# Enigmatisms/AdaPT

Measured on AMD Instinct MI355X. Metric: Msamples/s (W*H*spp/s), unidirectional MIS path tracing, higher is better.
Workload: dtype f32

## Files before the change

### adapt_amd/csrc/rng.hpp

```cpp
#pragma once
#include "vec.hpp"
#include <stdint.h>

struct Philox {
    uint32_t key0, key1, ctr0;
    uint32_t draw;
    uint32_t blk;
    uint32_t nblk;
    uint32_t c[4], n[4];
};

APT_HD void philox4x32_10(uint32_t c0, uint32_t c1, uint32_t c2, uint32_t c3, uint32_t k0, uint32_t k1, uint32_t out[4]) {
#if defined(__HIP_DEVICE_COMPILE__)
    asm volatile("" : "+v"(k0));
#endif
#pragma unroll
    for (int r = 0; r < 10; r++) {
        uint64_t p0 = (uint64_t)0xD2511F53u * c0;
        uint64_t p1 = (uint64_t)0xCD9E8D57u * c2;
        uint32_t n0 = (uint32_t)(p1 >> 32) ^ c1 ^ k0;
        uint32_t n1 = (uint32_t)p1;
        uint32_t n2 = (uint32_t)(p0 >> 32) ^ c3 ^ k1;
        uint32_t n3 = (uint32_t)p0;
        c0 = n0; c1 = n1; c2 = n2; c3 = n3;
        k0 += 0x9E3779B9u; k1 += 0xBB67AE85u;
    }
    out[0] = c0; out[1] = c1; out[2] = c2; out[3] = c3;
}

APT_HD void rng_init(Philox& r, uint32_t pixel, uint32_t seed, uint32_t sample, uint32_t draw) {
    r.key0 = pixel; r.key1 = seed; r.ctr0 = sample; r.draw = draw; r.blk = 0xffffffffu; r.nblk = 0xffffffffu;
    r.c[0] = r.c[1] = r.c[2] = r.c[3] = 0u;
    r.n[0] = r.n[1] = r.n[2] = r.n[3] = 0u;
}
APT_HD uint32_t rng_u32(Philox& r) {
    const uint32_t d = r.draw++;
    const uint32_t b = d >> 2;
    const bool step = b != r.blk;
    if (step && b != r.nblk) { philox4x32_10(r.ctr0, b, 0u, 0u, r.key0, r.key1, r.n); r.nblk = b; }
    if (step) { r.c[0] = r.n[0]; r.c[1] = r.n[1]; r.c[2] = r.n[2]; r.c[3] = r.n[3]; r.blk = b; r.nblk = 0xffffffffu; }
    const uint32_t w = d & 3u, c0 = r.c[0], c1 = r.c[1], c2 = r.c[2], c3 = r.c[3];
    return (w == 0u) ? c0 : ((w == 1u) ? c1 : ((w == 2u) ? c2 : c3));
}
APT_HD void rng_open(Philox& r) {
    const uint32_t b = r.draw >> 2;
    philox4x32_10(r.ctr0, b, 0u, 0u, r.key0, r.key1, r.c); r.blk = b;
    philox4x32_10(r.ctr0, b + 1u, 0u, 0u, r.key0, r.key1, r.n); r.nblk = b + 1u;
}
APT_HD float rng_float(Philox& r) { return (float)(rng_u32(r) >> 8) * (1.0f / 16777216.0f); }
APT_HD int32_t rng_int(Philox& r) { return (int32_t)rng_u32(r); }
APT_HD int pymod(int a, int n) { int m = a % n; return (m < 0) ? m + n : m; }
```

### adapt_amd/csrc/shade_stage.hpp

```cpp
#pragma once
#include "stages.hpp"

APT_D float ti_fmod(float a, float b) { float q = floorf(a / b); return a - b * q; }
APT_D f3 mix3(f3 a, f3 b, float t) { return a * (1.0f - t) + b * t; }
APT_D f3 texture_query(const DevScene& sc, int map, int obj, float u, float v) {
    const int* ti_ = sc.tex_i + 15 * obj + 5 * map; const float* tf = sc.tex_f + 6 * obj + 2 * map;
    const float w = (float)ti_[3], h = (float)ti_[4];
    const float scaled_u = ti_fmod((u * tf[0]) * w, w - 1.f), scaled_v = ti_fmod((v * tf[1]) * h, h - 1.f);
    float floor_u = floorf(scaled_u), floor_v = floorf(scaled_v);
    const float ratio_u = scaled_u - floor_u, ratio_v = scaled_v - floor_v;
    floor_u = floor_u + (float)ti_[1]; floor_v = floor_v + (float)ti_[2];
    const int fu = (int)floor_u, fv = (int)floor_v;
    const float* img = sc.atlas[map]; const int W = sc.atlas_w[map];
    const float* r0 = img + ((size_t)fv * W + fu) * 3; const float* r1 = r0 + (size_t)W * 3;
    const f3 q_ff = mk3(r0[0], r0[1], r0[2]), q_cf = mk3(r0[3], r0[4], r0[5]), q_fc = mk3(r1[0], r1[1], r1[2]), q_cc = mk3(r1[3], r1[4], r1[5]);
    return mix3(mix3(q_ff, q_cf, ratio_u), mix3(q_fc, q_cc, ratio_u), ratio_v);
}
APT_D bool get_uv_item(const DevScene& sc, int map, int obj, int prim, float bu, float bv, f3& out) {
    if (sc.atlas[map] == nullptr || !(sc.tex_i[15 * obj + 5 * map] > -255)) return false;
    const float* uv = sc.uvs + 6 * prim;
    const float w0 = 1.f - bu - bv;
    const float gu = (uv[2] * bu + uv[4] * bv) + uv[0] * w0, gv = (uv[3] * bu + uv[5] * bv) + uv[1] * w0;
    out = texture_query(sc, map, obj, gu, gv);
    return true;
// ... 83 lines not shown
    }
    flush_stat(t_lit, &cnt->stats[sq][ST_LIT]);
    if (lane_id() == 0) __hip_atomic_store(n_sh_p, 0u, __ATOMIC_RELAXED, __HIP_MEMORY_SCOPE_AGENT);
    __threadfence();
    if (lane_id() == 0) __hip_atomic_store(&cnt->fix_done[sq * CNT_PAD], epoch, __ATOMIC_RELEASE, __HIP_MEMORY_SCOPE_AGENT);
}
#endif
#ifndef APT_ARGS_RELOAD
#define APT_ARGS_RELOAD 1
#endif
struct ShadeArgs3 { DevScene sc; Params p; Queues q; };
typedef const __attribute__((address_space(4))) ShadeArgs3* args3_ptr;
APT_D args3_ptr kernel_args3() { return (args3_ptr)__builtin_amdgcn_kernarg_segment_ptr(); }
APT_D const ShadeArgs3* args_fresh(args3_ptr a) {
#if APT_ARGS_RELOAD
    asm volatile("" : "+s"(a));
#endif
    return (const ShadeArgs3*)a;
}
#if APT_ARGS_RELOAD
#define APT_ARGS_PHASE() (A_ = args_fresh(A0))
#else
#define APT_ARGS_PHASE() ((void)0)
#endif
struct Vertex {
    f3 o, d, thr, hit_point; uint32_t id, l_off, draw0; float emission_weight;
    Hit it; int hit_light; DevBxdf bx;
};
APT_D void vertex_reset(Vertex& vx) {
    vx.o = splat3(0.f); vx.d = mk3(0.f, 0.f, 1.f); vx.thr = splat3(0.f); vx.hit_point = splat3(0.f); vx.id = 0; vx.l_off = 0; vx.draw0 = 0; vx.emission_weight = 1.0f;
    vx.it.obj_id = -1; vx.it.prim_id = -1; vx.it.n_s = vx.it.n_g = mk3(1.f, 0.f, 0.f); vx.it.min_depth = 0.f; vx.hit_light = -1;
    vx.bx.type = 1; vx.bx.is_delta = 0; vx.bx.is_bsdf = 0; vx.bx.k_d = vx.bx.k_s = vx.bx.k_g = vx.bx.mean = splat3(0.f); vx.bx.ior = 1.f;
}
template <int BM, int SM, int TEX>
APT_D bool open_vertex(const ShadeArgs3* A_, Vertex& vx, Philox& rng, int prim, f3 rec_kd, uint32_t meta, float ray_pdf, float2 uv, int bounce) {
    const bool was_spec = (meta >> 24) & 1u;
    if (BM == 0x002) vx.bx.k_d = rec_kd;
    else vx.bx = ld_bxdf_lane((A_->sc).bxdf + vx.it.obj_id);
    if (TEX && (A_->sc).tex_i != nullptr) {
        f3 tx;
        if (bounce == 0) {
            if (get_uv_item((A_->sc), 1, vx.it.obj_id, prim, uv.x, uv.y, tx)) { m33 R; rotation_between(mk3(0.f, 1.f, 0.f), vx.it.n_g, R); vx.it.n_s = mul(R, tx); }
            if (get_uv_item((A_->sc), 2, vx.it.obj_id, prim, uv.x, uv.y, tx)) vx.it.n_s = delocalize(vx.it.n_s, tx);
        }
        if (get_uv_item((A_->sc), 0, vx.it.obj_id, prim, uv.x, uv.y, tx)) vx.bx.k_d = tx;
    }
    const uint32_t lp = vx.id & ((1u << (A_->p).pix_bits) - 1u), s = vx.id >> (A_->p).pix_bits;
    vx.l_off = (s * (uint32_t)(A_->p).npix + lp) << 2;
    vx.draw0 = meta & 0xffffu;
    rng_init(rng, ((A_->p).world == 1) ? lp : ldq((A_->p).pix_key, lp << 2), (A_->p).seed, (uint32_t)((A_->p).cnt_base + (int)s + 1), vx.draw0);
    if (bounce > 0 && (A_->p).use_mis) {
        float e_pdf = 0.0f;
        if (vx.hit_light >= 0 && vx.bx.is_delta == 0 && !was_spec) e_pdf = emitter_solid_angle_pdf((A_->sc).src[vx.hit_light], vx.it, vx.d);
        vx.emission_weight = balance(ray_pdf, e_pdf);
    }
    if (!(SM & 2)) rng_open(rng);
    if ((A_->p).use_rr) {
        float mx = max3(vx.thr);
        if (mx < (A_->p).rr_threshold && bounce >= (A_->p).rr_bounce_th) {
            if (rng_float(rng) > mx) return false;
            vx.thr = vx.thr * srcp(mx + 1e-7f);
        }
    } else if (max3(vx.thr) < 1e-4f) return false;
    return true;
}
struct LightSample { bool want, sampled, poisoned; f3 dir, contrib; float dist, mis_w; int src; };
template <int BM, int SM, bool LANE_SRC>
APT_D LightSample sample_light(const ShadeArgs3* A_, Vertex& vx, Philox& rng, const EmitterGeom& geom, const DevSrc src_only, bool active, bool& break_flag) {
    LightSample ls; ls.want = ls.sampled = ls.poisoned = false; ls.dir = ls.contrib = splat3(0.f); ls.dist = 0.f; ls.mis_w = 1.0f; ls.src = 0;
    if (!active || break_flag) return ls;
    const int ns = (A_->sc).n_sources;
    int sidx = rng_int(rng);
    sidx = (ns == 1) ? 0 : pymod(sidx, ns);
    float emitter_pdf = (A_->p).inv_ns;
    if (vx.hit_light >= 0) {
        if (ns <= 1) { break_flag = true; return ls; }
        sidx = rng_int(rng);
        sidx = (ns == 2) ? 0 : pymod(sidx, ns - 1);
        if (sidx >= vx.hit_light) sidx += 1;
        emitter_pdf = (A_->p).inv_ns1;
    }
    DevSrc src = src_only;
    if (ns != 1) src = LANE_SRC ? ld_src_lane((A_->sc).src + sidx) : (A_->sc).src[sidx];
    ls.src = sidx;
    f3 shadow_int; float direct_pdf;
    const f3 to_emitter = emitter_sample_hit<SM>(src, geom, vx.hit_point, rng, shadow_int, direct_pdf) - vx.hit_point;
    ls.dist = fnorm(to_emitter);
    ls.dir = fdiv3(to_emitter, ls.dist);
    ls.sampled = true;
    const f3 direct_spec = surface_eval<BM>(vx.bx, vx.it, vx.d, ls.dir, (A_->sc).world_ior, (A_->p).two_sides);
    if ((A_->p).use_mis && !(src.bool_bits & 0x01)) ls.mis_w = balance(emitter_pdf * direct_pdf, surface_pdf<BM>(vx.bx, vx.it, ls.dir, vx.d, (A_->sc).world_ior, (A_->p).two_sides));
    if (isnan(ls.mis_w)) { ls.poisoned = true; return ls; }
    f3 c = (direct_spec * shadow_int) * ls.mis_w;
    if (ns != 1) c = fdiv3(c, emitter_pdf);
    ls.contrib = (c * (A_->p).inv_S) * vx.thr;
    ls.want = !(ls.contrib.x == 0.f && ls.contrib.y == 0.f && ls.contrib.z == 0.f);
    return ls;
}
template <int BM, int SM, typename Gather>
APT_D f3 emit_and_scatter(const ShadeArgs3* A_, Vertex& vx, Philox& rng, float& new_pdf, bool& is_spec, Gather&& gather) {
    if ((SM & 2) && vx.hit_light >= 0) {
        const f3 emit_int = emitter_eval_le((A_->sc).src[vx.hit_light], vx.hit_point - vx.o, vx.it.n_s);
        if (!(emit_int.x == 0.f && emit_int.y == 0.f && emit_int.z == 0.f)) gather((emit_int * vx.emission_weight) * vx.thr);
    }
    f3 spec;
    const f3 new_d = surface_sample<BM>(vx.bx, vx.it, vx.d, (A_->sc).world_ior, (A_->p).two_sides, rng, spec, new_pdf, is_spec);
    vx.thr = vx.thr * fdiv3(spec, new_pdf);
    return new_d;
}
APT_D void shadow_store(const Queues& q, uint32_t so, f3 o, f3 dir, float dist, f3 contrib) {
    st3q(q.sh_o, q.sh_cap, so, o); st3q(q.sh_d, q.sh_cap, so, dir); stq(q.sh_tmax, so, dist); st3q(q.sh_c, q.sh_cap, so, contrib);
}
struct ShadeTally { uint32_t shade, shadow, poison; };
APT_D void tally_flush(const ShadeTally& t, const uint32_t* s_draws, Counters* cnt, int sq) {
    flush_uniform(t.shade, &cnt->stats[sq][ST_SHADE]);
    flush_uniform(t.shadow, &cnt->stats[sq][ST_SHADOW]);
    if (lane_id() == 0 && s_draws[threadIdx.x >> 6]) atomicAdd(&cnt->stats[sq][ST_DRAWS], (unsigned long long)s_draws[threadIdx.x >> 6]);
    flush_uniform(t.poison, &cnt->stats[sq][ST_POISON]);
}
#if APT_FAST
template <int BM, int SM, int TEX, bool CAM = false>
APT_D void shade_traced(args3_ptr A0, Counters* cnt, int cur_, int bounce_, const unsigned long long* strips = nullptr) {
    const ShadeArgs3* A_ = args_fresh(A0);
    const int cur = CAM ? 0 : cur_, bounce = CAM ? 0 : bounce_;
    const int nxt = cur ^ 1;
    const SubLoop sl = sub_loop((A_->p).nq);
    const uint32_t qbase = (uint32_t)sl.q * (A_->p).subcap, sh_qbase = (uint32_t)sl.q * (A_->q).sh_subcap;
    uint32_t* next_counter = &cnt->n_tr[(bounce + 1) % 3][0][sl.q * CNT_PAD];
    if (sl.first == 0 && threadIdx.x == 0) {
        cnt->n_tr[(bounce + 2) % 3][0][sl.q * CNT_PAD] = 0;
        cnt->n_tr[(bounce + 2) % 3][(A_->q).tr_ncls][sl.q * CNT_PAD] = 0;
    }
    const EmitterGeom geom = {(A_->sc).precom, (A_->sc).normals, (A_->sc).obj_info};
    __shared__ uint32_t s_draws[BLOCK / 64];
    if (lane_id() == 0) s_draws[threadIdx.x >> 6] = 0;
    ShadeTally tl = {0u, 0u, 0u};
    uint32_t t_traced = 0, t_lit = 0, t_extend = 0, t_samples = 0;
#ifdef APT_NEAR_STATS
    uint32_t t_near = 0;
#endif
    constexpr bool PFP = TEX == 0 && !CAM;
    static_assert(APT_FLAT_MAX_PRIMS < (int)TR_NO_PRIM, "the packed record keeps the hit primitive in 8 bits");
    const float4* trA = (A_->q).tr[cur][0]; const float4* trB = (A_->q).tr[cur][1]; const float4* trC = (A_->q).tr[cur][2]; const float4* trD = (A_->q).tr[cur][3];
    uint32_t n, cam_total = 0;
    if constexpr (CAM) {
        cam_total = (uint32_t)(A_->p).npix * (uint32_t)(A_->p).spp_batch;
        const uint32_t n_waves = (cam_total + 63u) / 64u, nq_ = (uint32_t)(A_->p).nq;
        n = n_waves > (uint32_t)sl.q ? ((n_waves - (uint32_t)sl.q + nq_ - 1u) / nq_) * 64u : 0u;
    } else {
        fix_prologue((A_->sc), (A_->p), (A_->q), cnt, cur, sl.q, bounce);
        n = __hip_atomic_load(&cnt->n_tr[bounce % 3][0][sl.q * CNT_PAD], __ATOMIC_RELAXED, __HIP_MEMORY_SCOPE_AGENT);
    }
    uint32_t pf_pm = 0;
    auto prefetch_prim = [&](uint32_t b) { pf_pm = ldq(reinterpret_cast<const uint32_t*>(trB), ((qbase + min(b + threadIdx.x, n - 1u)) << 4) + 12u); };
    if (PFP && n > 0) prefetch_prim(sl.first);
    for (uint32_t base = sl.first; base < n; base += sl.stride) {
        APT_ARGS_PHASE();
        const uint32_t pos = base + threadIdx.x, idx = qbase + pos;
        bool alive = pos < n;
        const uint32_t cu_pm = pf_pm;
        float4 cu_ra = make_float4(0.f, 0.f, 0.f, 0.f), cu_rb = cu_ra;
        if (PFP) { const int rp = max(tr_prim(cu_pm), 0); cu_ra = (A_->sc).prim_shade[2 * rp]; cu_rb = (A_->sc).prim_shade[2 * rp + 1]; prefetch_prim(base + sl.stride); }
        Vertex vx; vertex_reset(vx);
        Philox rng; rng_init(rng, 0u, 0u, 0u, 0u);
        f3 Lc = splat3(0.f);
        bool entry = alive;
        float ray_pdf = 1.f;
        if constexpr (CAM) {
            const uint32_t w = (uint32_t)__builtin_amdgcn_readfirstlane((int)(pos >> 6)) * (uint32_t)(A_->p).nq + (uint32_t)sl.q;
            const uint32_t id_ = w * 64u + lane_id();
            const bool valid = alive && id_ < cam_total;
            f3 dir = mk3(0.f, 0.f, 1.f);
            uint32_t draws = 0;
            if (valid) {
                const uint32_t lp = id_ % (uint32_t)(A_->p).npix, s = id_ / (uint32_t)(A_->p).npix;
                int i, j; local_to_global((A_->p), lp, i, j);
                for (int pl = 0; pl < (A_->p).l_planes; pl++) stL((A_->q).L, (A_->p).cap, (id_ << 2) | (uint32_t)pl, splat3(0.f));
                dir = camera_ray_dir((A_->p), i, j, s, draws);
                vx.id = (s << (A_->p).pix_bits) | lp;
            }
            if (draws) atomicAdd(&s_draws[threadIdx.x >> 6], draws);
            const f3 cam_o = mk3((A_->p).cam_t[0], (A_->p).cam_t[1], (A_->p).cam_t[2]);
            float c_t = 0.f; int c_run = -1, c_idx = -1;
            if (__any(valid)) c_idx = flat_closest1<true>((A_->sc).flat, cam_o, dir, 1e7f, c_t, c_run, camera_strip_mask((A_->p), strips, w));
            const bool c_defer = valid && (c_run >= 0 || flat_needs_cull((A_->sc).flat, dir));
            HitRec hr; hr.t = 1e7f; hr.prim = -1; hr.u = hr.v = 0.f;
            int hit_cls = 0;
            if (valid && !c_defer && c_idx >= 0) flat_resolve((A_->sc).flat, c_idx, c_t, cam_o, dir, hr, hit_cls);
            { const uint32_t nv = wave_count(valid); t_samples += nv; t_extend += nv; }
            if (__any(c_defer)) {
                const int ncls = (A_->q).tr_ncls;
                const uint32_t dpos = wave_append(c_defer, &cnt->n_tr[0][ncls][sl.q * CNT_PAD]);
                if (c_defer) {
                    const uint32_t slot = (A_->q).tr_stage_top ? qbase + (A_->p).subcap - 1u - dpos : (uint32_t)ncls * (A_->p).cap + qbase + dpos, so = slot << 4;
                    stq((A_->q).tr[0][0], so, make_float4(cam_o.x, cam_o.y, cam_o.z, hr.t));
                    stq((A_->q).tr[0][1], so, make_float4(dir.x, dir.y, dir.z, __uint_as_float(tr_pack(hr.prim, draws, false))));
                    stq((A_->q).tr[0][2], so, make_float4(1.f, 1.f, 1.f, __uint_as_float(vx.id)));
                    stq((A_->q).tr[0][3], so, make_float4(0.f, 0.f, 0.f, 1.f));
                    if ((A_->sc).has_vn || (A_->sc).tex_i != nullptr) { float2 uv_; uv_.x = hr.u; uv_.y = hr.v; stq((A_->q).tr_uv[0], slot << 3, uv_); }
                }
            }
            entry = valid && !c_defer;
            alive = entry && hr.prim >= 0;
            if (alive) {
                vx.o = cam_o; vx.d = dir; vx.thr = splat3(1.f);
                f3 rec_kd; float2 uv; uv.x = hr.u; uv.y = hr.v;
                build_hit((A_->sc), hr.prim, hr.t, uv.x, uv.y, vx.o, vx.d, vx.it, vx.hit_light, rec_kd);
                alive = open_vertex<BM, SM, TEX>(A_, vx, rng, hr.prim, rec_kd, tr_meta(tr_pack(hr.prim, draws, false), 0u), ray_pdf, uv, 0);
            }
        }
        if (!CAM && alive && bounce > 0) { const float4 dd = ldq(trD, idx << 4); Lc = mk3(dd.x, dd.y, dd.z); if (SM & 2) ray_pdf = dd.w; }
        if (!CAM && alive) {
            const float4 a = ldq(trA, idx << 4), b_ = ldq(trB, idx << 4), c = ldq(trC, idx << 4);
            vx.o = mk3(a.x, a.y, a.z); vx.d = mk3(b_.x, b_.y, b_.z); vx.thr = mk3(c.x, c.y, c.z); vx.id = __float_as_uint(c.w);
            const uint32_t pm = PFP ? cu_pm : __float_as_uint(b_.w);
            const int prim = tr_prim(pm);
            if (prim < 0) alive = false;
            else {
                f3 rec_kd; float2 uv; uv.x = uv.y = 0.f;
                if ((A_->sc).has_vn || (TEX && (A_->sc).tex_i != nullptr)) uv = ldq((A_->q).tr_uv[cur], idx << 3);
                if (PFP) build_hit_rec((A_->sc), cu_ra, cu_rb, prim, a.w, uv.x, uv.y, vx.o, vx.d, vx.it, vx.hit_light, rec_kd);
                else build_hit((A_->sc), prim, a.w, uv.x, uv.y, vx.o, vx.d, vx.it, vx.hit_light, rec_kd);
                alive = open_vertex<BM, SM, TEX>(A_, vx, rng, prim, rec_kd, tr_meta(pm, (uint32_t)bounce), ray_pdf, uv, bounce);
            }
        }
        tl.shade += wave_count(alive);
#ifdef APT_NEAR_STATS
        t_near += wave_count(alive && bounce > 0 && vx.it.min_depth < 2e-3f);
#endif
        if (alive) vx.hit_point = vx.d * vx.it.min_depth + vx.o;

        APT_ARGS_PHASE();
        bool break_flag = false;
        DevSrc src_only;
        if ((A_->sc).n_sources == 1) src_only = ld_src_uniform((A_->sc).src);
        const LightSample f = sample_light<BM, SM, false>(A_, vx, rng, geom, src_only, alive, break_flag);
        if (f.poisoned) Lc = splat3(f.mis_w);
        tl.shadow += wave_count(f.sampled); tl.poison += wave_count(f.poisoned);
        int occ_e = 0;
        if ((A_->sc).n_sources != 1) {
            const unsigned long long wm = __ballot(f.want);
// ... 247 lines not shown
```

### adapt_amd/csrc/shading.hpp

```cpp
#pragma once
#include "rng.hpp"
#include "vec.hpp"

#define BRDF_EPS 1e-7f

struct DevBxdf {
    int type, is_delta, is_bsdf, _pad;
    f3 k_d, k_s, k_g, mean;
    float ior;
    float _pad2[3];
};
struct DevSrc {
    int type, bool_bits, obj_ref_id;
    int prim_first;
    f3 intensity, dir, pos;
    float inv_area, r;
    int prim_count;
};
struct Hit {
    int obj_id, prim_id;
    f3 n_s, n_g;
    float min_depth;
};

// ... 33 lines not shown
    float d = dot(normal, ray);
    return normalize(ray - (normal * 2.f) * d);
}
APT_D f3 reflect_in(f3 ray, f3 normal, float& d) {
    d = dot(normal, ray);
    return normalize(ray - (normal * 2.f) * d);
}
APT_D float pow5(float x) { float x2 = x * x; float x4 = x2 * x2; return x * x4; }
APT_D f3 schlick(f3 r_s, float dot_val) {
    float p = pow5(1.f - dot_val);
    return r_s + mk3(1.f - r_s.x, 1.f - r_s.y, 1.f - r_s.z) * p;
}
APT_D float fresnel_dielectric(float n_in, float n_out, float cos_inc, float cos_ref) {
    float a = n_in * cos_inc, b = n_out * cos_inc, c = n_in * cos_ref, d = n_out * cos_ref;
    float rs = (a - d) / (a + d);
    float rp = (c - b) / (c + b);
    return 0.5f * (rs * rs + rp * rp);
}
APT_D bool total_reflection(float dot_normal, float ni, float nr) {
    return (1.f - sqr(ni / nr) * (1.f - sqr(dot_normal))) < 0.f;
}
APT_D f3 refract_snell(f3 incid, f3 normal, float dot_n, float ni, float nr, float& cos_r2) {
    float exiting = sgn(dot_n);
    float ratio = ni / nr;
    cos_r2 = 1.f - sqr(ratio) * (1.f - sqr(dot_n));
    if (cos_r2 > 0.f) return normalize((incid * ratio - normal * (ratio * dot_n)) + normal * (exiting * sqrtf(cos_r2)));
    return mk3(0.f, 0.f, 0.f);
}

APT_D f3 polar_dir(float cos_t, float sin_t, float phi) {
    float s, c; apt_sincos(phi, &s, &c);
    return mk3(c * sin_t, cos_t, s * sin_t);
}
APT_D f3 sample_cosine_hemisphere(Philox& r, float& pdf) {
    float eps = rng_float(r);
    float cos_t = ssqrt(eps), sin_t = ssqrt(1.f - eps);
    float phi = APT_2PI * rng_float(r);
    pdf = cos_t * APT_INV_PI;
    return polar_dir(cos_t, sin_t, phi);
}
APT_D f3 sample_mod_phong_lobe(Philox& r, float alpha, float& pdf) {
    float cos_t = apt_pow(rng_float(r), 1.f / (alpha + 1.f));
    float sin_t = ssqrt(1.f - cos_t * cos_t);
    float phi = APT_2PI * rng_float(r);
    pdf = 0.5f * (1.f + alpha) * apt_pow(cos_t, alpha) * APT_INV_PI;
    return polar_dir(cos_t, sin_t, phi);
}
APT_D f3 sample_uniform_sphere(Philox& r, float& pdf) {
    float cos_t = 2.f * rng_float(r) - 1.f;
    float sin_t = ssqrt(1.f - cos_t * cos_t);
    float phi = APT_2PI * rng_float(r);
    pdf = APT_INV_2PI * 0.5f;
    return polar_dir(cos_t, sin_t, phi);
}
APT_D f3 sample_fresnel_half(Philox& r, float nu, float nv, float& power_coeff) {
    float eps1 = rng_float(r) * 4.f;
    float inner = eps1 - floorf(eps1);
    float tan_phi = sqrtf((nu + 1.f) / (nv + 1.f)) * apt_tan(APT_PI_2 * inner);
    float cos_phi2 = 1.f / (1.f + tan_phi * tan_phi);
    float sin_phi2 = 1.f - cos_phi2;
    float cos_phi = sqrtf(cos_phi2);
    if (eps1 > 1.f && eps1 <= 3.f) cos_phi *= -1.f;
    float sin_phi = sqrtf(sin_phi2) * sgn(2.f - eps1);
    power_coeff = nu * cos_phi2 + nv * sin_phi2;
    float cos_t = apt_pow(1.f - rng_float(r), 1.f / (power_coeff + 1.f));
    float sin_t = ssqrt(1.f - cos_t * cos_t);
    return mk3(cos_phi * sin_t, cos_t, sin_phi * sin_t);
}
APT_D f3 sample_on_triangle(Philox& r, f3 dv1, f3 dv2) {
    float u1 = rng_float(r), u2 = rng_float(r);
    f3 pt = dv1 * u1 + dv2 * u2;
    if (u1 + u2 > 1.0f) pt = (dv1 + dv2) - pt;
    return pt;
}
APT_D float balance(float a, float b) { return (a > 1e-7f) ? sdiv(a, a + b) : 0.f; }

APT_D f3 lambert_eval(const DevBxdf& b, f3 normal, f3 out) {
    float c = fmaxf(0.f, dot(normal, out));
    return (b.k_d * APT_INV_PI) * c;
}
APT_D f3 lambert_sample(const DevBxdf& b, f3 normal, Philox& r, f3& spec, float& pdf) {
    f3 local = sample_cosine_hemisphere(r, pdf);
    f3 out = delocalize(normal, local);
    spec = lambert_eval(b, normal, out);
    return out;
}
template <int BM>
APT_D f3 blinn_phong_eval(const DevBxdf& b, const Hit& it, f3 in, f3 out) {
    float c = fmaxf(0.f, dot(it.n_s, out));
    if ((BM >> 11) & 1) return (b.k_d * APT_INV_PI) * c;
    f3 h = out - in;
    if (max3(abs3(h)) > BRDF_EPS) h = normalize(h); else h = splat3(0.f);
    float dc = fmaxf(0.f, dot(h, it.n_s));
    f3 glossy = pow_sv(dc, b.k_g);
    return ((b.k_d + b.k_s * (((b.k_g + 2.0f) * 0.5f) * glossy)) * APT_INV_PI) * c;
}
APT_D f3 mod_phong_eval(const DevBxdf& b, const Hit& it, f3 in, f3 out) {
    float dn = dot(it.n_s, out);
    f3 spec = splat3(0.f);
    if (dn > 0.f) {
        f3 refl = normalize((it.n_s * 2.f) * dn - out);
        float dv = fmaxf(0.f, -dot(in, refl));
        f3 glossy = pow_sv(dv, b.k_g) * b.k_s;
        spec = ((((b.k_g + 2.f) * 0.5f) * glossy) * APT_INV_PI) * dn;
        spec = spec + lambert_eval(b, it.n_s, out);
    }
    return spec;
}
APT_D f3 mod_phong_sample(const DevBxdf& b, const Hit& it, f3 incid, Philox& r, f3& spec, float& pdf) {
    float eps = rng_float(r);
    f3 out = mk3(0.f, 1.f, 0.f);
    spec = splat3(0.f);
    pdf = max3(b.k_d);
    float ks_max = max3(b.k_s);
// ... 222 lines not shown
        if (cos_o * cos_i < 0.f) {
            cos_i = fabsf(cos_i); cos_o = fabsf(cos_o);
            if (cos_o > BRDF_EPS && cos_i > BRDF_EPS) {
                spec = microfacet_eval_raw(b, it, half_vector, raw, incid, out_d) / (4.f * cos_o * cos_i);
                pdf = trow_reitz_pdf(-incid, half_vector, b.k_g, it.n_s);
                pdf /= 4.f * dot_val;
            }
        }
    }
    return out_d;
}

#define APT_BX_ALL 0x7ff
#define APT_SRC_ALL 0x17
#define BXHAS(M, bit) (((M) >> (bit)) & 1)

template <int BM>
APT_D f3 brdf_eval(const DevBxdf& b, const Hit& it, f3 incid, f3 out) {
    f3 ret = splat3(0.f);
    if (dot(incid, it.n_g) * dot(out, it.n_g) < 0.f) {
        switch (b.type) {
            case 0: if (BXHAS(BM, 0)) ret = blinn_phong_eval<BM>(b, it, incid, out); break;
            case 1: if (BXHAS(BM, 1)) ret = lambert_eval(b, it.n_s, out); break;
            case 4: if (BXHAS(BM, 4)) ret = mod_phong_eval(b, it, incid, out); break;
            case 5: if (BXHAS(BM, 5)) { m33 R; rotation_between(mk3(0.f, 1.f, 0.f), it.n_s, R); ret = fresnel_blend_eval(b, it, incid, out, R); } break;
            case 6: if (BXHAS(BM, 6)) ret = oren_nayar_eval(b, it, incid, out); break;
            case 7: if (BXHAS(BM, 7)) ret = thin_coat_eval(b, it, incid, out); break;
            case 3: if (BXHAS(BM, 3)) ret = microfacet_eval(b, it, incid, out); break;
            default: break;
        }
    }
    return ret;
}
template <int BM>
APT_D f3 brdf_sample(const DevBxdf& b, const Hit& it, f3 incid, Philox& r, f3& spec, float& pdf, bool& is_specular) {
    f3 dir = mk3(0.f, 1.f, 0.f);
    spec = splat3(1.f); pdf = 1.0f; is_specular = false;
    switch (b.type) {
        case 0: if (BXHAS(BM, 0)) {
            f3 local = sample_cosine_hemisphere(r, pdf);
            dir = delocalize(it.n_s, local);
            spec = blinn_phong_eval<BM>(b, it, incid, dir);
        } break;
        case 1: case 6: if (BXHAS(BM, 1) || BXHAS(BM, 6)) dir = lambert_sample(b, it.n_s, r, spec, pdf); break;
        case 2: if (BXHAS(BM, 2)) { dir = reflect_in(incid, it.n_s); spec = b.k_d; pdf = 1.0f; } break;
        case 7: if (BXHAS(BM, 7)) dir = thin_coat_sample(b, it, incid, r, spec, pdf, is_specular); break;
        case 4: if (BXHAS(BM, 4)) dir = mod_phong_sample(b, it, incid, r, spec, pdf); break;
        case 5: if (BXHAS(BM, 5)) dir = fresnel_blend_sample(b, it, incid, r, spec, pdf); break;
        case 3: if (BXHAS(BM, 3)) dir = microfacet_sample(b, it, incid, r, spec, pdf); break;
        default: break;
    }
    if (!(dot(dir, it.n_g) > 0.f)) spec = splat3(0.f);
    return dir;
}
template <int BM>
APT_D float brdf_pdf(const DevBxdf& b, const Hit& it, f3 outdir, f3 incid) {
    float pdf = 0.f;
    float d_out = dot(it.n_s, outdir);
    float d_in = dot(it.n_s, incid);
    if (d_out * d_in < 0.f) {
        switch (b.type) {
            case 0: case 1: case 6: pdf = d_out * APT_INV_PI; break;
            case 4: if (BXHAS(BM, 4)) {
                float g = b.mean.z;
                f3 rv = reflect_in(incid, it.n_s);
                float dro = fmaxf(0.f, dot(rv, outdir));
                float dpdf = d_out * APT_INV_PI;
                float spdf = 0.5f * (g + 1.f) * APT_INV_PI * apt_pow(dro, g);
                pdf = max3(b.k_d) * dpdf + max3(b.k_s) * spdf;
            } break;
            case 7: if (BXHAS(BM, 7)) {
                f3 refl = reflect_in(incid, it.n_s);
                float F = thin_coat_fresnel(b, it, incid);
                pdf = (fabsf(dot(outdir, refl)) > (1.f - 1e-3f)) ? F : (1.f - F) * d_out * APT_INV_PI;
            } break;
            case 5: if (BXHAS(BM, 5)) {
                f3 h = normalize(outdir - incid);
                float d_half = dot(h, it.n_s);
                m33 R; rotation_between(mk3(0.f, 1.f, 0.f), it.n_s, R);
                float c2, s2; fb_cos2_sin2(h, it.n_s, R, d_half, c2, s2);
                pdf = b.k_g.z * apt_pow(d_half, b.k_g.x * c2 + b.k_g.y * s2) / fabsf(dot(incid, h));
                pdf = 0.5f * (pdf + d_out * APT_INV_PI);
// ... 88 lines not shown
    } else {
        float ratio = ni / nr;
        float cos_r2 = 1.f - sqr(ratio) * (1.f - sqr(d_out));
        float d_in = dot(in, it.n_s);
        if (cos_r2 > 0.f) {
            float F = fresnel_dielectric(ni, nr, fabsf(d_out), sqrtf(cos_r2));
            if (d_in * d_out < 0.f) { if (dot(ref_dir, in) > 1.f - 1e-4f) ret = b.k_d * F; }
            else ret = b.k_d * ((1.f - F) * APT_INV_PI * fabsf(d_out));
        } else if (dot(ref_dir, in) > 1.f - 1e-4f) ret = b.k_d;
    }
    return ret;
}
APT_D float bsdf_pdf(const DevBxdf& b, const Hit& it, f3 outdir, f3 incid, float world_ior) {
    float pdf = 0.f;
    if (b.type == -1) return (dot(incid, outdir) > 1.f - 1e-4f) ? 1.f : 0.f;
    float d_out = dot(outdir, it.n_s);
    bool entering = d_out < 0.f;
    float ni = entering ? world_ior : b.ior, nr = entering ? b.ior : world_ior;
    f3 ref_dir = normalize(outdir - (it.n_s * 2.f) * d_out);
    float cos_r2;
    f3 refra = refract_snell(outdir, it.n_s, d_out, ni, nr, cos_r2);
    if (cos_r2 > 0.0f) {
        float F = fresnel_dielectric(ni, nr, fabsf(d_out), sqrtf(cos_r2));
        if (dot(ref_dir, incid) > 1.f - 1e-4f) pdf = F;
        else if (b.type == 0 && dot(refra, incid) > 1.f - 1e-4f) pdf = 1.f - F;
        else if (b.type == 1 && (dot(incid, it.n_s) * d_out > 0.f)) pdf = (1.f - F) * fabsf(d_out) * APT_INV_PI;
    } else if (dot(ref_dir, incid) > 1.f - 1e-4f) pdf = 1.f;
    return pdf;
}

APT_D void flip_if_two_sided(Hit& it, f3 incid, int two_sides) {
    if (two_sides && dot(incid, it.n_s) > 0.f) { it.n_s = -it.n_s; it.n_g = -it.n_g; }
}
template <int BM>
APT_D f3 surface_sample(const DevBxdf& b, Hit& it, f3 incid, float world_ior, int two_sides, Philox& r, f3& spec, float& pdf, bool& is_specular) {
    if (!(BM & 0x700) || !b.is_bsdf) { flip_if_two_sided(it, incid, two_sides); return brdf_sample<BM>(b, it, incid, r, spec, pdf, is_specular); }
    spec = splat3(0.f); pdf = 0.f; is_specular = false;
    if (BXHAS(BM, 8) && b.type == 0) return glass_sample(b, it, incid, world_ior, r, spec, pdf);
    if (BXHAS(BM, 9) && b.type == 1) return lambert_trans_sample(b, it, incid, world_ior, r, spec, pdf, is_specular);
    return splat3(0.f);
}
template <int BM>
APT_D f3 surface_eval(const DevBxdf& b, Hit& it, f3 incid, f3 out, float world_ior, int two_sides) {
    if (!(BM & 0x700) || !b.is_bsdf) { flip_if_two_sided(it, incid, two_sides); return brdf_eval<BM>(b, it, incid, out); }
    if (BXHAS(BM, 8) && b.type == 0) return glass_eval(b, it, incid, out, world_ior);
    if (BXHAS(BM, 9) && b.type == 1) return lambert_trans_eval(b, it, incid, out, world_ior);
    return splat3(0.f);
}
template <int BM>
APT_D float surface_pdf(const DevBxdf& b, Hit& it, f3 outdir, f3 incid, float world_ior, int two_sides) {
    if (!(BM & 0x700) || !b.is_bsdf) { flip_if_two_sided(it, incid, two_sides); return brdf_pdf<BM>(b, it, outdir, incid); }
    return bsdf_pdf(b, it, outdir, incid, world_ior);
}

struct EmitterGeom {
    const float* precom;
    const float* normals;
    const int* obj_info;
};
APT_D f3 ld3(const float* p) { return mk3(p[0], p[1], p[2]); }

template <int SM>
APT_D f3 emitter_sample_hit(const DevSrc& s, const EmitterGeom& g, f3 hit_pos, Philox& r, f3& inten, float& pdf) {
    inten = s.intensity;
    f3 pos = s.pos;
    pdf = 1.0f;
    if (BXHAS(SM, 0) && s.type == 0) {
        f3 x = hit_pos - pos;
        inten = inten * fminf(srcp(fmaxf(norm2(x), 1e-5f)), 1.0f);
    } else if (BXHAS(SM, 1) && s.type == 1) {
        pdf = s.inv_area;
        f3 normal;
        if (s.prim_count < 0) {
            const float* pc = g.precom + 9 * s.prim_first;
            f3 center = ld3(pc);
            float radius = pc[3];
            f3 to_hit = normalize(hit_pos - center);
            float p;
            f3 local = sample_uniform_sphere(r, p);
            normal = delocalize(to_hit, local);
            pos = center + normal * radius;
            pdf = sdiv(p, radius * radius);
        } else {
            int tri = pymod(rng_int(r), s.prim_count) + s.prim_first;
            normal = ld3(g.normals + 3 * tri);
            const float* pc = g.precom + 9 * tri;
            pos = sample_on_triangle(r, ld3(pc), ld3(pc + 3)) + ld3(pc + 6);
        }
        f3 diff = hit_pos - pos;
        float dl = dot(fnormalize(diff), normal);
        if (dl <= 0.0f) { inten = splat3(0.f); pdf = 1.0f; }
        else {
            pdf *= sdiv(norm2(diff), dl);
            inten = (pdf > 0.0f) ? fdiv3(inten, pdf) : splat3(0.f);
        }
    } else if (BXHAS(SM, 2) && s.type == 2) {
        f3 to_hit = hit_pos - pos;
        float depth = fmaxf(fnorm(to_hit), 1e-5f);
        to_hit = fdiv3(to_hit, depth);
        if (dot(to_hit, s.dir) > s.r) inten = fdiv3(inten, depth * depth);
        else inten = splat3(0.f);
    } else if (BXHAS(SM, 4) && s.type == 4) {
        pdf = 0.f;
        if (s.r > 0.f) {
            f3 to_hit = hit_pos - s.pos;
            float proj = dot(to_hit, s.dir);
            if (proj > 0.0f) {
                float dist = ssqrt(norm2(to_hit) - proj * proj);
                if (dist < s.r) pos = hit_pos - s.dir * proj;
                else inten = splat3(0.f);
            }
        } else inten = splat3(0.f);
    }
    return pos;
}
APT_D f3 emitter_eval_le(const DevSrc& s, f3 inci_dir, f3 normal) {
    if (s.type == 1 && -dot(normalize(inci_dir), normal) > 0.f) return s.intensity;
    return splat3(0.f);
}
APT_D float emitter_solid_angle_pdf(const DevSrc& s, const Hit& it, f3 incid_dir) {
    float d = fabsf(dot(incid_dir, it.n_s));
    float area_pdf = (s.type == 1) ? s.inv_area : 0.f;
    return (d > 0.0f) ? sdiv(area_pdf * sqr(it.min_depth), d) : 0.0f;
}
```

### adapt_amd/csrc/stages.hpp

```cpp
#pragma once
#include <hip/hip_runtime.h>

#include "rng.hpp"
#include "shading.hpp"
#include "traverse.hpp"
#include "vec.hpp"

struct DevMedium {
    int type;
    float ior;
    f3 u_s, u_a, u_e, par, pdf;
};
struct DevVolume {
    int type, xres, yres, zres;
    f3 albedo, trans, mini, maxi, majorant, pdf;
    f3 inv_r0, inv_r1, inv_r2;
    DevMedium ph;
    const float* grid;
};
struct DevScene {
    DevBvh bvh;
    SweepScene sweep;
    FlatScene flat;
    const float* normals;
// ... 234 lines not shown
    DevBxdf x;
    x.type = __float_as_int(a.x); x.is_delta = __float_as_int(a.y); x.is_bsdf = __float_as_int(a.z); x._pad = 0;
    x.k_d = mk3(b.x, b.y, b.z); x.k_s = mk3(b.w, c.x, c.y); x.k_g = mk3(c.z, c.w, d.x); x.mean = mk3(d.y, d.z, d.w);
    x.ior = e.x; x._pad2[0] = x._pad2[1] = x._pad2[2] = 0.f;
    return x;
#else
    return *p;
#endif
}

APT_D void local_to_global(const Params& p, uint32_t lp, int& i, int& j) {
    int lc = (int)(lp / (uint32_t)p.H);
    j = (int)(lp % (uint32_t)p.H);
    int lb = lc / p.band_width, w = lc % p.band_width;
    i = (lb * p.world + p.rank) * p.band_width + w;
}

struct SubLoop { int q; uint32_t first, stride; };
APT_D SubLoop sub_loop(int nq, int nt = BLOCK) {
    SubLoop s;
    s.q = (int)(blockIdx.x % (uint32_t)nq);
    s.first = (blockIdx.x / (uint32_t)nq) * (uint32_t)nt;
    s.stride = (gridDim.x / (uint32_t)nq) * (uint32_t)nt;
    return s;
}
#ifndef APT_TILE_NT
#define APT_TILE_NT 512
#endif
#ifndef APT_TILE_WAVES
#define APT_TILE_WAVES 6
#endif
#define TRACE_NT(MODE) ((MODE) == 2 ? APT_TILE_NT : BLOCK)

APT_D f3 camera_ray_dir(const Params& p, int i, int j, uint32_t s, uint32_t& draws) {
    int sample_cnt = p.cnt_base + (int)s + 1;
    Philox rng; rng_init(rng, (uint32_t)(i * p.H + j), p.seed, (uint32_t)sample_cnt, 0u);
    float vx = 0.5f, vy = 0.5f;
    if (p.anti_alias) {
        if (p.stratified) {
            int mod_val = pymod(sample_cnt, 16);
            vx = (float)(mod_val % 4) * 0.25f + rng_float(rng) * 0.25f;
            vy = (float)(mod_val / 4) * 0.25f + rng_float(rng) * 0.25f;
        } else {
            const float eps = 1e-4f, inv_eps = (float)(1 - 1e-4 * 2.);
            vx = rng_float(rng) * inv_eps + eps;
            vy = rng_float(rng) * inv_eps + eps;
        }
    }
    f3 cd = mk3((p.half_w + vx - (float)i) * p.inv_focal, ((float)j - p.half_h - vy) * p.inv_focal, 1.f);
    m33 R;
    for (int a = 0; a < 3; a++) for (int b = 0; b < 3; b++) R.m[a][b] = p.cam_r[3 * a + b];
    draws = rng.draw;
    return normalize(mul(R, cd));
}
APT_D unsigned long long camera_strip_mask(const Params& p, const unsigned long long* strips, uint32_t w) {
    typedef const __attribute__((address_space(4))) unsigned long long* strip_ptr;
    const uint32_t lp0 = (uint32_t)__builtin_amdgcn_readfirstlane((int)((w * 64u) % (uint32_t)p.npix)), lp1 = lp0 + 63u, last = (uint32_t)p.npix - 1u;
    return ((strip_ptr)strips)[lp0 >> 6] | ((strip_ptr)strips)[(lp1 < last ? lp1 : last) >> 6] | ((strip_ptr)strips)[lp1 > last ? 0u : (lp0 >> 6)];
}

template <bool TRACE, bool ADAPTIVE = false>
APT_D void generate_body(const DevScene* sc, const Params& p, const Queues& q, Counters* cnt, const uint8_t* active = nullptr, const unsigned long long* strips = nullptr) {
    const uint32_t total = (uint32_t)p.npix * (uint32_t)p.spp_batch;
    const uint32_t n_waves = (total + 63u) / 64u;
    const uint32_t wave_stride = gridDim.x * (BLOCK / 64);
    uint32_t t_samples = 0, t_draws = 0;
    for (uint32_t w = blockIdx.x * (BLOCK / 64) + threadIdx.x / 64u; w < n_waves; w += wave_stride) {
        const uint32_t idx = w * 64u + lane_id();
        const int sq = (int)(w % (uint32_t)p.nq);
        bool valid = idx < total, alive = false;
        f3 dir = mk3(0.f, 0.f, 1.f);
        uint32_t draws = 0;
        if (valid) {
            uint32_t lp = idx % (uint32_t)p.npix, s = idx / (uint32_t)p.npix;
            int i, j; local_to_global(p, lp, i, j);
            for (int pl = 0; pl < p.l_planes; pl++) stL(q.L, p.cap, (idx << 2) | (uint32_t)pl, splat3(0.f));
            alive = !p.do_crop || (i >= p.sx && i < p.ex && j >= p.sy && j < p.ey);
            if (ADAPTIVE) alive = alive && active[lp] != 0;
            if (alive) {
                dir = camera_ray_dir(p, i, j, s, draws);
            }
        }
        uint32_t pos;
        uint32_t* q0_counter = &cnt->n_active[0][sq * CNT_PAD];
        if (TRACE) pos = 0;
// ... 651 lines not shown
```

Measured before the change: 6051.

## Add a draw-window RNG that precomputes each vertex's Philox words for Lambertian shading

Adds a DrawWindow RNG type for Lambertian-only, non-emitting shader variants. It computes the Philox block once at vertex open and serves the roulette, light-index and two hemisphere draws from preselected words. The second Philox block is evaluated only when some lane in the wave needs it. On camera bounces the first block is reused from the jitter computation's leftover words, so the per-vertex Philox work and the per-draw branching are meant to shrink. The change also turns several BSDF and emitter branches into if-constexpr so unused material code is not compiled in. The risk is that the word-selection logic must reproduce the exact old random stream, and the camera-tail reuse only holds when the jitter used the same counter block.

```diff
diff --git a/adapt_amd/csrc/rng.hpp b/adapt_amd/csrc/rng.hpp
--- a/adapt_amd/csrc/rng.hpp
+++ b/adapt_amd/csrc/rng.hpp
@@ -1,6 +1,7 @@
 #pragma once
 #include "vec.hpp"
 #include <stdint.h>
+#include <type_traits>
 
 struct Philox {
     uint32_t key0, key1, ctr0;
@@ -49,4 +50,43 @@
 }
 APT_HD float rng_float(Philox& r) { return (float)(rng_u32(r) >> 8) * (1.0f / 16777216.0f); }
 APT_HD int32_t rng_int(Philox& r) { return (int32_t)rng_u32(r); }
+
+#ifndef APT_DRAW_WINDOW
+#define APT_DRAW_WINDOW 1
+#endif
+#ifndef APT_DRAW_WINDOW_CARRY
+#define APT_DRAW_WINDOW_CARRY 1
+#endif
+struct DrawWindow {
+    uint32_t draw;
+    uint32_t e, u[2];
+    uint32_t rr;
+};
+APT_HD void rng_init(DrawWindow& w, uint32_t, uint32_t, uint32_t, uint32_t draw) { w.draw = draw; w.e = w.u[0] = w.u[1] = w.rr = 0u; }
+APT_HD float window_unit(uint32_t w) { return (float)(w >> 8) * (1.0f / 16777216.0f); }
+APT_HD bool window_spans(uint32_t s) { return s + 2u >= 4u; }
+template <typename Any>
+APT_HD bool window_open(DrawWindow& w, uint32_t key0, uint32_t key1, uint32_t ctr0, uint32_t d0, bool roulette, float mx, bool relight,
+                        uint32_t c[4], bool have_first, Any&& any) {
+    const uint32_t b = d0 >> 2, off = d0 & 3u;
+    if (!have_first) philox4x32_10(ctr0, b, 0u, 0u, key0, key1, c);
+    const uint32_t c0 = c[0], c1 = c[1], c2 = c[2], c3 = c[3];
+    w.draw = d0; w.rr = 0u;
+    bool live = true;
+    if (roulette) {
+        w.rr = (off & 2u) ? ((off & 1u) ? c3 : c2) : ((off & 1u) ? c1 : c0);
+        w.draw = d0 + 1u;
+        live = !(window_unit(w.rr) > mx);
+    }
+    const uint32_t s = off + (roulette ? 1u : 0u) + (relight ? 1u : 0u);
+    uint32_t n[4] = {0u, 0u, 0u, 0u};
+    if (any(live && window_spans(s))) philox4x32_10(ctr0, b + 1u, 0u, 0u, key0, key1, n);
+    const bool hi = (s & 4u) != 0u, b1 = (s & 2u) != 0u, b0 = (s & 1u) != 0u;
+    const uint32_t x0 = hi ? n[0] : c0, x1 = hi ? n[1] : c1, x2 = hi ? n[2] : c2, x3 = hi ? n[3] : c3;
+    const uint32_t y0 = b1 ? x2 : x0, y1 = b1 ? x3 : x1, y2 = b1 ? n[0] : x2, y3 = b1 ? n[1] : x3;
+    w.e = b0 ? y1 : y0; w.u[0] = b0 ? y2 : y1; w.u[1] = b0 ? y3 : y2;
+    return live;
+}
+APT_HD int32_t rng_int(DrawWindow& w) { w.draw++; return (int32_t)w.e; }
+APT_HD float rng_float(DrawWindow& w) { const uint32_t v = w.u[0]; w.u[0] = w.u[1]; w.draw++; return window_unit(v); }
 APT_HD int pymod(int a, int n) { int m = a % n; return (m < 0) ? m + n : m; }
diff --git a/adapt_amd/csrc/shade_stage.hpp b/adapt_amd/csrc/shade_stage.hpp
--- a/adapt_amd/csrc/shade_stage.hpp
+++ b/adapt_amd/csrc/shade_stage.hpp
@@ -139,8 +139,8 @@
     vx.it.obj_id = -1; vx.it.prim_id = -1; vx.it.n_s = vx.it.n_g = mk3(1.f, 0.f, 0.f); vx.it.min_depth = 0.f; vx.hit_light = -1;
     vx.bx.type = 1; vx.bx.is_delta = 0; vx.bx.is_bsdf = 0; vx.bx.k_d = vx.bx.k_s = vx.bx.k_g = vx.bx.mean = splat3(0.f); vx.bx.ior = 1.f;
 }
-template <int BM, int SM, int TEX>
-APT_D bool open_vertex(const ShadeArgs3* A_, Vertex& vx, Philox& rng, int prim, f3 rec_kd, uint32_t meta, float ray_pdf, float2 uv, int bounce) {
+template <int BM, int SM, int TEX, typename RNG>
+APT_D bool open_vertex(const ShadeArgs3* A_, Vertex& vx, RNG& rng, int prim, f3 rec_kd, uint32_t meta, float ray_pdf, float2 uv, int bounce, const uint32_t* jitter_tail = nullptr) {
     const bool was_spec = (meta >> 24) & 1u;
     if (BM == 0x002) vx.bx.k_d = rec_kd;
     else vx.bx = ld_bxdf_lane((A_->sc).bxdf + vx.it.obj_id);
@@ -155,25 +155,39 @@
     const uint32_t lp = vx.id & ((1u << (A_->p).pix_bits) - 1u), s = vx.id >> (A_->p).pix_bits;
     vx.l_off = (s * (uint32_t)(A_->p).npix + lp) << 2;
     vx.draw0 = meta & 0xffffu;
-    rng_init(rng, ((A_->p).world == 1) ? lp : ldq((A_->p).pix_key, lp << 2), (A_->p).seed, (uint32_t)((A_->p).cnt_base + (int)s + 1), vx.draw0);
+    const uint32_t key0 = ((A_->p).world == 1) ? lp : ldq((A_->p).pix_key, lp << 2), ctr0 = (uint32_t)((A_->p).cnt_base + (int)s + 1);
+    rng_init(rng, key0, (A_->p).seed, ctr0, vx.draw0);
     if (bounce > 0 && (A_->p).use_mis) {
         float e_pdf = 0.0f;
         if (vx.hit_light >= 0 && vx.bx.is_delta == 0 && !was_spec) e_pdf = emitter_solid_angle_pdf((A_->sc).src[vx.hit_light], vx.it, vx.d);
         vx.emission_weight = balance(ray_pdf, e_pdf);
     }
-    if (!(SM & 2)) rng_open(rng);
-    if ((A_->p).use_rr) {
-        float mx = max3(vx.thr);
-        if (mx < (A_->p).rr_threshold && bounce >= (A_->p).rr_bounce_th) {
-            if (rng_float(rng) > mx) return false;
-            vx.thr = vx.thr * srcp(mx + 1e-7f);
-        }
-    } else if (max3(vx.thr) < 1e-4f) return false;
-    return true;
+    if constexpr (std::is_same<RNG, DrawWindow>::value) {
+        static_assert(BM == 0x002 && !(SM & 2), "a draw window serves [roulette] index [index] u1 u2: Lambertian surfaces, emitters that draw nothing");
+        bool roulette = false; float mx = 0.f;
+        if ((A_->p).use_rr) { mx = max3(vx.thr); roulette = mx < (A_->p).rr_threshold && bounce >= (A_->p).rr_bounce_th; }
+        else if (max3(vx.thr) < 1e-4f) return false;
+        const bool relight = vx.hit_light >= 0 && (A_->sc).n_sources > 1;
+        const bool have_first = jitter_tail != nullptr && (A_->p).anti_alias != 0;
+        uint32_t c[4] = {0u, 0u, have_first ? jitter_tail[0] : 0u, have_first ? jitter_tail[1] : 0u};
+        if (!window_open(rng, key0, (A_->p).seed, ctr0, vx.draw0, roulette, mx, relight, c, have_first, [](bool v) { return __any(v) != 0; })) return false;
+        if (roulette) vx.thr = vx.thr * srcp(mx + 1e-7f);
+        return true;
+    } else {
+        if (!(SM & 2)) rng_open(rng);
+        if ((A_->p).use_rr) {
+            float mx = max3(vx.thr);
+            if (mx < (A_->p).rr_threshold && bounce >= (A_->p).rr_bounce_th) {
+                if (rng_float(rng) > mx) return false;
+                vx.thr = vx.thr * srcp(mx + 1e-7f);
+            }
+        } else if (max3(vx.thr) < 1e-4f) return false;
+        return true;
+    }
 }
 struct LightSample { bool want, sampled, poisoned; f3 dir, contrib; float dist, mis_w; int src; };
-template <int BM, int SM, bool LANE_SRC>
-APT_D LightSample sample_light(const ShadeArgs3* A_, Vertex& vx, Philox& rng, const EmitterGeom& geom, const DevSrc src_only, bool active, bool& break_flag) {
+template <int BM, int SM, bool LANE_SRC, typename R>
+APT_D LightSample sample_light(const ShadeArgs3* A_, Vertex& vx, R& rng, const EmitterGeom& geom, const DevSrc src_only, bool active, bool& break_flag) {
     LightSample ls; ls.want = ls.sampled = ls.poisoned = false; ls.dir = ls.contrib = splat3(0.f); ls.dist = 0.f; ls.mis_w = 1.0f; ls.src = 0;
     if (!active || break_flag) return ls;
     const int ns = (A_->sc).n_sources;
@@ -204,8 +218,8 @@
     ls.want = !(ls.contrib.x == 0.f && ls.contrib.y == 0.f && ls.contrib.z == 0.f);
     return ls;
 }
-template <int BM, int SM, typename Gather>
-APT_D f3 emit_and_scatter(const ShadeArgs3* A_, Vertex& vx, Philox& rng, float& new_pdf, bool& is_spec, Gather&& gather) {
+template <int BM, int SM, typename R, typename Gather>
+APT_D f3 emit_and_scatter(const ShadeArgs3* A_, Vertex& vx, R& rng, float& new_pdf, bool& is_spec, Gather&& gather) {
     if ((SM & 2) && vx.hit_light >= 0) {
         const f3 emit_int = emitter_eval_le((A_->sc).src[vx.hit_light], vx.hit_point - vx.o, vx.it.n_s);
         if (!(emit_int.x == 0.f && emit_int.y == 0.f && emit_int.z == 0.f)) gather((emit_int * vx.emission_weight) * vx.thr);
@@ -246,6 +260,8 @@
 #ifdef APT_NEAR_STATS
     uint32_t t_near = 0;
 #endif
+    constexpr bool WINDOW = APT_DRAW_WINDOW != 0 && BM == 0x002 && !(SM & 2);
+    typedef typename std::conditional<WINDOW, DrawWindow, Philox>::type Rng;
     constexpr bool PFP = TEX == 0 && !CAM;
     static_assert(APT_FLAT_MAX_PRIMS < (int)TR_NO_PRIM, "the packed record keeps the hit primitive in 8 bits");
     const float4* trA = (A_->q).tr[cur][0]; const float4* trB = (A_->q).tr[cur][1]; const float4* trC = (A_->q).tr[cur][2]; const float4* trD = (A_->q).tr[cur][3];
@@ -269,7 +285,7 @@
         float4 cu_ra = make_float4(0.f, 0.f, 0.f, 0.f), cu_rb = cu_ra;
         if (PFP) { const int rp = max(tr_prim(cu_pm), 0); cu_ra = (A_->sc).prim_shade[2 * rp]; cu_rb = (A_->sc).prim_shade[2 * rp + 1]; prefetch_prim(base + sl.stride); }
         Vertex vx; vertex_reset(vx);
-        Philox rng; rng_init(rng, 0u, 0u, 0u, 0u);
+        Rng rng; rng_init(rng, 0u, 0u, 0u, 0u);
         f3 Lc = splat3(0.f);
         bool entry = alive;
         float ray_pdf = 1.f;
@@ -279,11 +295,12 @@
             const bool valid = alive && id_ < cam_total;
             f3 dir = mk3(0.f, 0.f, 1.f);
             uint32_t draws = 0;
+            uint32_t jitter_tail[2] = {0u, 0u};
             if (valid) {
                 const uint32_t lp = id_ % (uint32_t)(A_->p).npix, s = id_ / (uint32_t)(A_->p).npix;
                 int i, j; local_to_global((A_->p), lp, i, j);
                 for (int pl = 0; pl < (A_->p).l_planes; pl++) stL((A_->q).L, (A_->p).cap, (id_ << 2) | (uint32_t)pl, splat3(0.f));
-                dir = camera_ray_dir((A_->p), i, j, s, draws);
+                dir = camera_ray_dir((A_->p), i, j, s, draws, (WINDOW && APT_DRAW_WINDOW_CARRY) ? jitter_tail : nullptr);
                 vx.id = (s << (A_->p).pix_bits) | lp;
             }
             if (draws) atomicAdd(&s_draws[threadIdx.x >> 6], draws);
@@ -303,7 +320,9 @@
                     stq((A_->q).tr[0][0], so, make_float4(cam_o.x, cam_o.y, cam_o.z, hr.t));
                     stq((A_->q).tr[0][1], so, make_float4(dir.x, dir.y, dir.z, __uint_as_float(tr_pack(hr.prim, draws, false))));
                     stq((A_->q).tr[0][2], so, make_float4(1.f, 1.f, 1.f, __uint_as_float(vx.id)));
-                    stq((A_->q).tr[0][3], so, make_float4(0.f, 0.f, 0.f, 1.f));
+                    float one = 1.f;
+                    if (WINDOW) asm volatile("" : "+v"(one));
+                    stq((A_->q).tr[0][3], so, make_float4(0.f, 0.f, 0.f, one));
                     if ((A_->sc).has_vn || (A_->sc).tex_i != nullptr) { float2 uv_; uv_.x = hr.u; uv_.y = hr.v; stq((A_->q).tr_uv[0], slot << 3, uv_); }
                 }
             }
@@ -313,7 +332,7 @@
                 vx.o = cam_o; vx.d = dir; vx.thr = splat3(1.f);
                 f3 rec_kd; float2 uv; uv.x = hr.u; uv.y = hr.v;
                 build_hit((A_->sc), hr.prim, hr.t, uv.x, uv.y, vx.o, vx.d, vx.it, vx.hit_light, rec_kd);
-                alive = open_vertex<BM, SM, TEX>(A_, vx, rng, hr.prim, rec_kd, tr_meta(tr_pack(hr.prim, draws, false), 0u), ray_pdf, uv, 0);
+                alive = open_vertex<BM, SM, TEX>(A_, vx, rng, hr.prim, rec_kd, tr_meta(tr_pack(hr.prim, draws, false), 0u), ray_pdf, uv, 0, (WINDOW && APT_DRAW_WINDOW_CARRY) ? jitter_tail : nullptr);
             }
         }
         if (!CAM && alive && bounce > 0) { const float4 dd = ldq(trD, idx << 4); Lc = mk3(dd.x, dd.y, dd.z); if (SM & 2) ray_pdf = dd.w; }
diff --git a/adapt_amd/csrc/shading.hpp b/adapt_amd/csrc/shading.hpp
--- a/adapt_amd/csrc/shading.hpp
+++ b/adapt_amd/csrc/shading.hpp
@@ -89,7 +89,8 @@
     float s, c; apt_sincos(phi, &s, &c);
     return mk3(c * sin_t, cos_t, s * sin_t);
 }
-APT_D f3 sample_cosine_hemisphere(Philox& r, float& pdf) {
+template <typename R>
+APT_D f3 sample_cosine_hemisphere(R& r, float& pdf) {
     float eps = rng_float(r);
     float cos_t = ssqrt(eps), sin_t = ssqrt(1.f - eps);
     float phi = APT_2PI * rng_float(r);
@@ -136,7 +137,8 @@
     float c = fmaxf(0.f, dot(normal, out));
     return (b.k_d * APT_INV_PI) * c;
 }
-APT_D f3 lambert_sample(const DevBxdf& b, f3 normal, Philox& r, f3& spec, float& pdf) {
+template <typename R>
+APT_D f3 lambert_sample(const DevBxdf& b, f3 normal, R& r, f3& spec, float& pdf) {
     f3 local = sample_cosine_hemisphere(r, pdf);
     f3 out = delocalize(normal, local);
     spec = lambert_eval(b, normal, out);
@@ -425,22 +427,22 @@
     }
     return ret;
 }
-template <int BM>
-APT_D f3 brdf_sample(const DevBxdf& b, const Hit& it, f3 incid, Philox& r, f3& spec, float& pdf, bool& is_specular) {
+template <int BM, typename R>
+APT_D f3 brdf_sample(const DevBxdf& b, const Hit& it, f3 incid, R& r, f3& spec, float& pdf, bool& is_specular) {
     f3 dir = mk3(0.f, 1.f, 0.f);
     spec = splat3(1.f); pdf = 1.0f; is_specular = false;
     switch (b.type) {
-        case 0: if (BXHAS(BM, 0)) {
+        case 0: if constexpr (BXHAS(BM, 0)) {
             f3 local = sample_cosine_hemisphere(r, pdf);
             dir = delocalize(it.n_s, local);
             spec = blinn_phong_eval<BM>(b, it, incid, dir);
         } break;
-        case 1: case 6: if (BXHAS(BM, 1) || BXHAS(BM, 6)) dir = lambert_sample(b, it.n_s, r, spec, pdf); break;
-        case 2: if (BXHAS(BM, 2)) { dir = reflect_in(incid, it.n_s); spec = b.k_d; pdf = 1.0f; } break;
-        case 7: if (BXHAS(BM, 7)) dir = thin_coat_sample(b, it, incid, r, spec, pdf, is_specular); break;
-        case 4: if (BXHAS(BM, 4)) dir = mod_phong_sample(b, it, incid, r, spec, pdf); break;
-        case 5: if (BXHAS(BM, 5)) dir = fresnel_blend_sample(b, it, incid, r, spec, pdf); break;
-        case 3: if (BXHAS(BM, 3)) dir = microfacet_sample(b, it, incid, r, spec, pdf); break;
+        case 1: case 6: if constexpr (BXHAS(BM, 1) || BXHAS(BM, 6)) dir = lambert_sample(b, it.n_s, r, spec, pdf); break;
+        case 2: if constexpr (BXHAS(BM, 2)) { dir = reflect_in(incid, it.n_s); spec = b.k_d; pdf = 1.0f; } break;
+        case 7: if constexpr (BXHAS(BM, 7)) dir = thin_coat_sample(b, it, incid, r, spec, pdf, is_specular); break;
+        case 4: if constexpr (BXHAS(BM, 4)) dir = mod_phong_sample(b, it, incid, r, spec, pdf); break;
+        case 5: if constexpr (BXHAS(BM, 5)) dir = fresnel_blend_sample(b, it, incid, r, spec, pdf); break;
+        case 3: if constexpr (BXHAS(BM, 3)) dir = microfacet_sample(b, it, incid, r, spec, pdf); break;
         default: break;
     }
     if (!(dot(dir, it.n_g) > 0.f)) spec = splat3(0.f);
@@ -595,12 +597,14 @@
 APT_D void flip_if_two_sided(Hit& it, f3 incid, int two_sides) {
     if (two_sides && dot(incid, it.n_s) > 0.f) { it.n_s = -it.n_s; it.n_g = -it.n_g; }
 }
-template <int BM>
-APT_D f3 surface_sample(const DevBxdf& b, Hit& it, f3 incid, float world_ior, int two_sides, Philox& r, f3& spec, float& pdf, bool& is_specular) {
+template <int BM, typename R>
+APT_D f3 surface_sample(const DevBxdf& b, Hit& it, f3 incid, float world_ior, int two_sides, R& r, f3& spec, float& pdf, bool& is_specular) {
     if (!(BM & 0x700) || !b.is_bsdf) { flip_if_two_sided(it, incid, two_sides); return brdf_sample<BM>(b, it, incid, r, spec, pdf, is_specular); }
-    spec = splat3(0.f); pdf = 0.f; is_specular = false;
-    if (BXHAS(BM, 8) && b.type == 0) return glass_sample(b, it, incid, world_ior, r, spec, pdf);
-    if (BXHAS(BM, 9) && b.type == 1) return lambert_trans_sample(b, it, incid, world_ior, r, spec, pdf, is_specular);
+    if constexpr ((BM & 0x700) != 0) {
+        spec = splat3(0.f); pdf = 0.f; is_specular = false;
+        if (BXHAS(BM, 8) && b.type == 0) return glass_sample(b, it, incid, world_ior, r, spec, pdf);
+        if (BXHAS(BM, 9) && b.type == 1) return lambert_trans_sample(b, it, incid, world_ior, r, spec, pdf, is_specular);
+    }
     return splat3(0.f);
 }
 template <int BM>
@@ -623,15 +627,15 @@
 };
 APT_D f3 ld3(const float* p) { return mk3(p[0], p[1], p[2]); }
 
-template <int SM>
-APT_D f3 emitter_sample_hit(const DevSrc& s, const EmitterGeom& g, f3 hit_pos, Philox& r, f3& inten, float& pdf) {
+template <int SM, typename R>
+APT_D f3 emitter_sample_hit(const DevSrc& s, const EmitterGeom& g, f3 hit_pos, R& r, f3& inten, float& pdf) {
     inten = s.intensity;
     f3 pos = s.pos;
     pdf = 1.0f;
     if (BXHAS(SM, 0) && s.type == 0) {
         f3 x = hit_pos - pos;
         inten = inten * fminf(srcp(fmaxf(norm2(x), 1e-5f)), 1.0f);
-    } else if (BXHAS(SM, 1) && s.type == 1) {
+    } else if (BXHAS(SM, 1) && s.type == 1) { if constexpr (BXHAS(SM, 1)) {
         pdf = s.inv_area;
         f3 normal;
         if (s.prim_count < 0) {
@@ -657,7 +661,7 @@
             pdf *= sdiv(norm2(diff), dl);
             inten = (pdf > 0.0f) ? fdiv3(inten, pdf) : splat3(0.f);
         }
-    } else if (BXHAS(SM, 2) && s.type == 2) {
+    } } else if (BXHAS(SM, 2) && s.type == 2) {
         f3 to_hit = hit_pos - pos;
         float depth = fmaxf(fnorm(to_hit), 1e-5f);
         to_hit = fdiv3(to_hit, depth);
diff --git a/adapt_amd/csrc/stages.hpp b/adapt_amd/csrc/stages.hpp
--- a/adapt_amd/csrc/stages.hpp
+++ b/adapt_amd/csrc/stages.hpp
@@ -290,7 +290,7 @@
 #endif
 #define TRACE_NT(MODE) ((MODE) == 2 ? APT_TILE_NT : BLOCK)
 
-APT_D f3 camera_ray_dir(const Params& p, int i, int j, uint32_t s, uint32_t& draws) {
+APT_D f3 camera_ray_dir(const Params& p, int i, int j, uint32_t s, uint32_t& draws, uint32_t* tail = nullptr) {
     int sample_cnt = p.cnt_base + (int)s + 1;
     Philox rng; rng_init(rng, (uint32_t)(i * p.H + j), p.seed, (uint32_t)sample_cnt, 0u);
     float vx = 0.5f, vy = 0.5f;
@@ -309,6 +309,7 @@
     m33 R;
     for (int a = 0; a < 3; a++) for (int b = 0; b < 3; b++) R.m[a][b] = p.cam_r[3 * a + b];
     draws = rng.draw;
+    if (tail) { tail[0] = rng.c[2]; tail[1] = rng.c[3]; }
     return normalize(mul(R, cd));
 }
 APT_D unsigned long long camera_strip_mask(const Params& p, const unsigned long long* strips, uint32_t w) {
```

Result: faster. 6185, median of 6 (+2.2%).
